# JARVIS-MoCap/JARVIS-HybridNet

Hardware: AMD Instinct MI355X
Metric: multi-view frames/s (12cam 1280x1024, 23kpt, 64^3 grid) (higher is better)
Workload: dtype f32; 1 GPU; BASELINE configs[2]: HybridNet 12-camera 1280x1024, 23 kpts, 64^3 grid, small/small; cameras=12, joints=23, grid=64, streams=3, parallelism=single GPU, 3 time batches in flight on 3 HIP streams, hipgraph=False

## Files before the change

include/jarvis_hip.h:

```cpp
#ifndef JARVIS_HIP_H
#define JARVIS_HIP_H
#include <stdint.h>

#ifdef __cplusplus
extern "C" {
#endif

#define JH_ABI_VERSION 4

const char* jh_last_error(void);
int jh_abi_version(void);

#define JH_PRECISION_DEFAULT (-1)
#define JH_PRECISION_F32 0
#define JH_PRECISION_BF16X3 1
#define JH_PRECISION_BF16X3_WIDE 2
int jh_set_precision(int mode);
int jh_get_precision(void);

typedef struct jh_params jh_params;
int jh_params_create(jh_params** out);
int jh_params_set(jh_params* p, const char* key, const float* host, int64_t numel);
void jh_params_destroy(jh_params* p);

typedef struct jh_efftrack jh_efftrack;
int jh_efftrack_create(const jh_params* p, const char* prefix, int model_size, int joints, int n,
                       int h, int w, int want_res1, jh_efftrack** out);
int jh_efftrack_forward(jh_efftrack* net, const float* x_dev, float* res1_dev, float* res2_dev,
                        void* stream);
int64_t jh_efftrack_launches(const jh_efftrack* net);
void jh_efftrack_destroy(jh_efftrack* net);

typedef struct jh_v2v jh_v2v;
int jh_v2v_create(const jh_params* p, const char* prefix, int joints, int t, int g, jh_v2v** out);
int jh_v2v_forward(jh_v2v* net, const float* x_dev, float* y_dev, void* stream);
void jh_v2v_destroy(jh_v2v* net);
int jh_v2v_fold(int joints, int t, int g, int* folded);

int64_t jh_reproject_workspace_bytes(int cams, int joints, int hs, int grid_size);
int jh_reproject_forward(const float* heatmaps_padded_dev, int cams, int joints, int hs,
                         const int32_t* center3d_dev, const int32_t* center_hm_dev,
                         const float* cam_dev, const float* intr_dev, const float* dist_dev,
                         int grid_size, float grid_spacing, float* vol_dev, int32_t* idx_dev,
                         void* workspace_dev, int64_t workspace_bytes, void* stream);

int64_t jh_softargmax_workspace_bytes(int t, int joints, int gh);
int jh_softargmax(const float* v2v_out_dev, int t, int joints, int gh, float grid_spacing,
                  float roi_cube_size, const int32_t* center3d_dev, float* heatmap_final_dev,
                  float* points_dev, float* conf_dev, void* workspace_dev, int64_t workspace_bytes,
                  void* stream);

int jh_reproject_point(const float* points_dev, int npoints, int cams, const float* cam_dev,
                       const float* intr_dev, const float* dist_dev, float* uv_dev, void* stream);
int64_t jh_reconstruct_workspace_bytes(int cams);
int jh_reconstruct_point(const float* points2d_dev, const float* maxvals_dev, int cams,
                         const float* cam_dev, const float* intr_dev, const float* dist_dev,
                         float* point3d_dev, void* workspace_dev, int64_t workspace_bytes,
                         void* stream);

typedef struct jh_predictor jh_predictor;
typedef struct {
  int32_t num_cameras, num_joints;
  int32_t center_size;
  int32_t bbox;
  float roi_cube_size;
  float grid_spacing;
  int32_t center_model, kp_model;
  int32_t img_h, img_w;
  int32_t time_batch;
  int32_t time_batch_3d;
  int32_t cam_lo, cam_n;
  float mean[3], std[3];
  int32_t precision;
} jh_predictor_config;

int jh_predictor_create(const jh_params* center_params, const jh_params* hybrid_params,
                        const jh_predictor_config* cfg, jh_predictor** out);
void jh_predictor_destroy(jh_predictor* pr);
int64_t jh_predictor_launches(const jh_predictor* pr);
int64_t jh_predictor_device_bytes(const jh_predictor* pr);
int jh_predictor_precision(const jh_predictor* pr);

int jh_predictor_set_calibration(jh_predictor* pr, const float* cam_dev, const float* intr_dev,
                                 const float* dist_dev, void* stream);
int jh_predictor_set_calibration_frames(jh_predictor* pr, const float* cam_dev ,
                                        const float* intr_dev , const float* dist_dev ,
                                        void* stream);

int jh_predictor_set_centers(jh_predictor* pr, const float* centers_dev , void* stream);

// ... 193 lines not shown
```

jarvis-hybridnet_amd/_native.py:

```python
import ctypes
import math
import os
from typing import NamedTuple

import torch

_HERE = os.path.dirname(os.path.abspath(__file__))
LIB_PATH = os.environ.get("JH_LIBRARY_PATH") or os.path.join(_HERE, "libjarvis_hip.so")
_lib = None

c_void_p, c_int, c_float, c_int64 = ctypes.c_void_p, ctypes.c_int, ctypes.c_float, ctypes.c_int64
c_char_p = ctypes.c_char_p


class PredictorConfig(ctypes.Structure):
    _fields_ = [("num_cameras", ctypes.c_int32), ("num_joints", ctypes.c_int32),
                ("center_size", ctypes.c_int32), ("bbox", ctypes.c_int32),
                ("roi_cube_size", c_float), ("grid_spacing", c_float),
                ("center_model", ctypes.c_int32), ("kp_model", ctypes.c_int32),
                ("img_h", ctypes.c_int32), ("img_w", ctypes.c_int32),
                ("time_batch", ctypes.c_int32), ("time_batch_3d", ctypes.c_int32),
                ("cam_lo", ctypes.c_int32),
                ("cam_n", ctypes.c_int32), ("mean", c_float * 3), ("std", c_float * 3),
                ("precision", ctypes.c_int32)]
# ... 13 lines not shown
    _fields_ = [("image_stride", ctypes.c_int64), ("offset", ctypes.c_int64), ("pitch", ctypes.c_int64),
                ("pattern", ctypes.c_int32), ("reserved", ctypes.c_int32)]


assert ctypes.sizeof(SensorSurfaceStruct) == 32

class OpOperand(ctypes.Structure):
    _fields_ = [("in_sums_host", c_void_p), ("in_act", ctypes.c_int32), ("latency_class", ctypes.c_int32),
                ("want_stats", ctypes.c_int32), ("se_c", ctypes.c_int32), ("se_s", ctypes.c_int32),
                ("se_inv_hw", c_float), ("se_wr_host", c_void_p), ("se_br_host", c_void_p),
                ("se_we_host", c_void_p), ("se_be_host", c_void_p), ("se_pool_host", c_void_p)]


assert ctypes.sizeof(OpOperand) == 72

class SubjectsParamsStruct(ctypes.Structure):
    _fields_ = [("max_subjects", ctypes.c_int32), ("max_peaks", ctypes.c_int32), ("nms_radius", ctypes.c_int32),
                ("min_views", ctypes.c_int32), ("min_peak", c_float), ("max_error_px", c_float)]


assert ctypes.sizeof(SubjectsParamsStruct) == 24

ABI_VERSION = 4
assert ctypes.sizeof(PredictorConfig) == 84

_WORKSPACES = {}


def workspace(nbytes, device):
    key = (str(device), torch.cuda.current_stream(device).cuda_stream)
    bufs = _WORKSPACES.setdefault(key, [])
    if not bufs or bufs[-1].numel() < nbytes:
        bufs.append(torch.empty((max(int(nbytes), 256),), dtype=torch.uint8, device=device))
    return bufs[-1]


_SIGS = {
    "jh_last_error": (c_char_p, []),
    "jh_abi_version": (c_int, []),
    "jh_set_precision": (c_int, [c_int]),
    "jh_get_precision": (c_int, []),
    "jh_params_create": (c_int, [ctypes.POINTER(c_void_p)]),
    "jh_params_set": (c_int, [c_void_p, c_char_p, c_void_p, c_int64]),
    "jh_params_destroy": (None, [c_void_p]),
    "jh_efftrack_create": (c_int, [c_void_p, c_char_p, c_int, c_int, c_int, c_int, c_int, c_int,
                                   ctypes.POINTER(c_void_p)]),
    "jh_efftrack_forward": (c_int, [c_void_p, c_void_p, c_void_p, c_void_p, c_void_p]),
    "jh_efftrack_launches": (c_int64, [c_void_p]),
    "jh_efftrack_destroy": (None, [c_void_p]),
    "jh_v2v_create": (c_int, [c_void_p, c_char_p, c_int, c_int, c_int, ctypes.POINTER(c_void_p)]),
    "jh_v2v_forward": (c_int, [c_void_p, c_void_p, c_void_p, c_void_p]),
    "jh_v2v_destroy": (None, [c_void_p]),
    "jh_v2v_fold": (c_int, [c_int, c_int, c_int, ctypes.POINTER(c_int)]),
    "jh_reproject_workspace_bytes": (c_int64, [c_int, c_int, c_int, c_int]),
    "jh_reproject_forward": (c_int, [c_void_p, c_int, c_int, c_int, c_void_p, c_void_p, c_void_p,
                                     c_void_p, c_void_p, c_int, c_float, c_void_p, c_void_p,
                                     c_void_p, c_int64, c_void_p]),
    "jh_softargmax_workspace_bytes": (c_int64, [c_int, c_int, c_int]),
    "jh_softargmax": (c_int, [c_void_p, c_int, c_int, c_int, c_float, c_float, c_void_p, c_void_p,
                              c_void_p, c_void_p, c_void_p, c_int64, c_void_p]),
    "jh_softargmax_spread_workspace_bytes": (c_int64, [c_int, c_int, c_int]),
    "jh_softargmax_spread": (c_int, [c_void_p, c_int, c_int, c_int, c_float, c_float, c_void_p, c_void_p,
                                     c_void_p, c_void_p, c_void_p, c_void_p, c_void_p, c_void_p, c_int64, c_void_p]),
    "jh_predictor_set_spread": (c_int, [c_void_p, c_int]),
    "jh_predictor_get_spread": (c_int, [c_void_p, c_void_p, c_void_p, c_void_p, c_void_p]),
    "jh_predictor_debug_v2v": (c_int, [c_void_p, c_void_p, c_void_p]),
    "jh_reproject_point": (c_int, [c_void_p, c_int, c_int, c_void_p, c_void_p, c_void_p, c_void_p,
                                   c_void_p]),
    "jh_reconstruct_workspace_bytes": (c_int64, [c_int]),
    "jh_reconstruct_point": (c_int, [c_void_p, c_void_p, c_int, c_void_p, c_void_p, c_void_p,
                                     c_void_p, c_void_p, c_int64, c_void_p]),
    "jh_predictor_create": (c_int, [c_void_p, c_void_p, ctypes.POINTER(PredictorConfig),
                                    ctypes.POINTER(c_void_p)]),
    "jh_predictor_destroy": (None, [c_void_p]),
    "jh_predictor_set_graph_replay": (c_int, [c_void_p, c_int]),
    "jh_predictor_graph_replay": (c_int, [c_void_p]),
    "jh_predictor_launches": (c_int64, [c_void_p]),
    "jh_predictor_device_bytes": (c_int64, [c_void_p]),
    "jh_predictor_precision": (c_int, [c_void_p]),
    "jh_predictor_set_calibration": (c_int, [c_void_p, c_void_p, c_void_p, c_void_p, c_void_p]),
    "jh_predictor_set_calibration_frames": (c_int, [c_void_p, c_void_p, c_void_p, c_void_p, c_void_p]),
    "jh_predictor_set_centers": (c_int, [c_void_p, c_void_p, c_void_p]),
    "jh_predictor_stage_center": (c_int, [c_void_p, c_void_p, c_void_p, c_void_p]),
    "jh_predictor_stage_keypoints": (c_int, [c_void_p, c_void_p, c_void_p, c_void_p, c_void_p]),
    "jh_predictor_stage_3d": (c_int, [c_void_p, c_void_p, c_int, c_void_p, c_void_p, c_void_p,
                                      c_void_p]),
    "jh_predictor_stage_keypoints_gathered": (c_int, [c_void_p, c_void_p, c_int, c_void_p, c_int, c_void_p,
                                                      c_void_p]),
    "jh_predictor_stage_3d_blocks": (c_int, [c_void_p, c_void_p, c_int, c_int, c_int, c_int, c_void_p,
                                             c_void_p, c_void_p, c_void_p]),
    "jh_profile_begin": (c_int, []),
    "jh_profile_end": (c_int, [ctypes.POINTER(c_int)]),
    "jh_profile_get": (c_int, [c_int, c_char_p, c_int, ctypes.POINTER(ctypes.c_double),
                               ctypes.POINTER(ctypes.c_double), ctypes.POINTER(ctypes.c_double)]),
    "jh_predictor_forward": (c_int, [c_void_p, c_void_p, c_void_p, c_void_p, c_void_p, c_void_p]),
    "jh_predictor_stage_center_u8": (c_int, [c_void_p, c_void_p, c_void_p, c_void_p]),
    "jh_predictor_stage_keypoints_u8": (c_int, [c_void_p, c_void_p, c_void_p, c_void_p, c_void_p]),
    "jh_predictor_forward_u8": (c_int, [c_void_p, c_void_p, c_void_p, c_void_p, c_void_p, c_void_p]),
    "jh_predictor_forward_yuv": (c_int, [c_void_p, c_void_p, c_int, c_void_p, c_void_p, c_void_p, c_void_p]),
    "jh_yuv_surface_check": (c_int, [ctypes.POINTER(YuvSurfaceStruct), c_int, c_int]),
    "jh_predictor_forward_surface": (c_int, [c_void_p, c_void_p, ctypes.POINTER(YuvSurfaceStruct), c_void_p, c_void_p,
                                             c_void_p, c_void_p, c_void_p]),
    "jh_predictor2d_forward_surface": (c_int, [c_void_p, c_void_p, ctypes.POINTER(YuvSurfaceStruct), c_void_p,
                                               c_void_p, c_void_p, c_void_p]),
    "jh_op_yuv_surface_to_bgr": (c_int, [c_void_p, ctypes.POINTER(YuvSurfaceStruct), c_int, c_int, c_int, c_void_p,
                                         c_void_p]),
# ... 402 lines not shown
```

jarvis-hybridnet_amd/csrc/api.hip:

```cpp
#include <cstring>
#include <memory>
#include "../../include/jarvis_hip.h"
#include <cstdlib>
#include "nets.h"
#include "bifpn_node.h"
#include "views2d.h"
#include "subjects.h"

namespace jh {
static thread_local std::string g_err;
void set_error(const std::string& msg) { g_err = msg; }
}

using namespace jh;

struct jh_params { ParamMap map; };
struct jh_efftrack { EffTrackPlan plan; };
struct jh_v2v { V2VPlan plan; };

namespace {

struct Scratch {
  std::vector<void*> ptrs;
  ~Scratch() { for (void* p : ptrs) (void)hipFree(p); }
// ... 126 lines not shown
  return 0;
}
int jh_get_precision(void) { return precision_mode(); }

int jh_params_create(jh_params** out) {
  *out = new jh_params();
  return 0;
}
int jh_params_set(jh_params* p, const char* key, const float* host, int64_t numel) {
  JH_REQUIRE(p && key && host && numel >= 0, "bad argument");
  p->map[key] = std::vector<float>(host, host + numel);
  return 0;
}
void jh_params_destroy(jh_params* p) { delete p; }

int jh_efftrack_create(const jh_params* p, const char* prefix, int model_size, int joints, int n,
                       int h, int w, int want_res1, jh_efftrack** out) {
  JH_REQUIRE(p && out, "bad argument");
  std::unique_ptr<jh_efftrack> net(new jh_efftrack());
  if (net->plan.build(p->map, prefix ? prefix : "", model_size, joints, n, h, w, want_res1 != 0)) return 1;
  *out = net.release();
  return 0;
}
int jh_efftrack_forward(jh_efftrack* net, const float* x_dev, float* res1_dev, float* res2_dev,
                        void* stream) {
  hipStream_t s = static_cast<hipStream_t>(stream);
  JH_REQUIRE(net && x_dev && res2_dev, "bad argument");
  JH_REQUIRE(!res1_dev || net->plan.res1.p, "res1 requested from a network created with want_res1 = 0");
  if (launch_to_channel_last(x_dev, net->plan.input, s)) return 1;
  if (net->plan.run(s)) return 1;
  if (res1_dev && launch_from_channel_last(net->plan.res1, res1_dev, s)) return 1;
  return launch_from_channel_last(net->plan.heat, res2_dev, s);
}
int64_t jh_efftrack_launches(const jh_efftrack* net) { return (int64_t)net->plan.launches(); }
void jh_efftrack_destroy(jh_efftrack* net) { delete net; }

int jh_v2v_create(const jh_params* p, const char* prefix, int joints, int t, int g, jh_v2v** out) {
  JH_REQUIRE(p && out, "bad argument");
  std::unique_ptr<jh_v2v> net(new jh_v2v());
  if (net->plan.build(p->map, prefix ? prefix : "", joints, t, g)) return 1;
  *out = net.release();
  return 0;
}
int jh_v2v_forward(jh_v2v* net, const float* x_dev, float* y_dev, void* stream) {
  hipStream_t s = static_cast<hipStream_t>(stream);
  if (launch_to_channel_last(x_dev, net->plan.input, s)) return 1;
  if (net->plan.run(s)) return 1;
  return launch_from_channel_last(net->plan.output, y_dev, s);
}
void jh_v2v_destroy(jh_v2v* net) { delete net; }
int jh_v2v_fold(int joints, int t, int g, int* folded) {
  JH_REQUIRE(joints >= 1 && t >= 1 && g >= 4 && g % 4 == 0 && folded, "jh_v2v_fold: bad argument");
  *folded = v2v_fold_applies(joints, g) ? 1 : 0;
  return 0;
}

int64_t jh_reproject_workspace_bytes(int cams, int joints, int hs, int grid_size) {
  Carver c(nullptr, 0);
  ReproWs w;
  return (int64_t)carve_reproject(c, cams, joints, hs, grid_size, &w);
}

int jh_reproject_forward(const float* heatmaps_padded_dev, int cams, int joints, int hs,
                         const int32_t* center3d_dev, const int32_t* center_hm_dev,
                         const float* cam_dev, const float* intr_dev, const float* dist_dev,
                         int grid_size, float grid_spacing, float* vol_dev, int32_t* idx_dev,
                         void* workspace_dev, int64_t workspace_bytes, void* stream) {
  hipStream_t s = static_cast<hipStream_t>(stream);
  JH_REQUIRE(workspace_dev && workspace_bytes >= 0, "workspace (see jh_reproject_workspace_bytes)");
  JH_REQUIRE(grid_size > 0 && grid_size % 2 == 0, "grid size must be even");
  Carver c(workspace_dev, (size_t)workspace_bytes);
  ReproWs w;
  carve_reproject(c, cams, joints, hs, grid_size, &w);
  JH_REQUIRE(c.fits(), "workspace smaller than jh_reproject_workspace_bytes()");
  if (launch_to_channel_last(heatmaps_padded_dev, w.heat, s)) return 1;
  if (launch_reproject(Calib{cam_dev, intr_dev, dist_dev, 0}, center3d_dev, center_hm_dev, w.heat.p, w.coarse,
                       w.vol.p, idx_dev, 1, cams, grid_size, grid_spacing, hs, w.heat.Cp,
                       1, 0, nullptr, s)) return 1;
  return launch_from_channel_last(w.vol, vol_dev, s);
}

int64_t jh_softargmax_workspace_bytes(int t, int joints, int gh) {
  Carver c(nullptr, 0);
  SoftWs w;
  return (int64_t)carve_softargmax(c, t, joints, gh, &w);
}

int jh_softargmax(const float* v2v_out_dev, int t, int joints, int gh, float grid_spacing,
                  float roi_cube_size, const int32_t* center3d_dev, float* heatmap_final_dev,
                  float* points_dev, float* conf_dev, void* workspace_dev, int64_t workspace_bytes,
                  void* stream) {
  hipStream_t s = static_cast<hipStream_t>(stream);
  JH_REQUIRE(workspace_dev && workspace_bytes >= 0, "workspace (see jh_softargmax_workspace_bytes)");
  Carver c(workspace_dev, (size_t)workspace_bytes);
  SoftWs w;
  carve_softargmax(c, t, joints, gh, &w);
  JH_REQUIRE(c.fits(), "workspace smaller than jh_softargmax_workspace_bytes()");
  if (launch_to_channel_last(v2v_out_dev, w.x, s)) return 1;
  return launch_softargmax(w.x.p, center3d_dev, w.partial, w.pmax, points_dev, conf_dev,
                           heatmap_final_dev, t, joints, w.x.Cp, gh, grid_spacing, roi_cube_size, s);
}

int64_t jh_softargmax_spread_workspace_bytes(int t, int joints, int gh) {
  Carver c(nullptr, 0);
  SoftWs w;
  SoftargmaxSpread sp;
// ... 1440 lines not shown
```

jarvis-hybridnet_amd/csrc/conv_host.hip:

```cpp
#include <vector>
#include <cstring>
#include <algorithm>
#include "conv_mfma.h"

namespace jh {

ConvDesc conv_desc(int nd, int k, int stride, int pad, int cin, int cout) {
  ConvDesc d{};
  d.nd = nd; d.k = k; d.stride = stride; d.ostride = 1; d.nphase = 1;
  d.cin = cin; d.cout = cout;
  d.phase[0].pad[0] = (nd == 3) ? pad : 0;
  d.phase[0].pad[1] = pad; d.phase[0].pad[2] = pad;
  d.phase[0].ooff[0] = d.phase[0].ooff[1] = d.phase[0].ooff[2] = 0;
  return d;
}

ConvDesc deconv2d_k4s2p1_desc(int cin, int cout) {
  ConvDesc d{};
  d.nd = 2; d.k = 2; d.stride = 1; d.ostride = 2; d.nphase = 4;
  d.cin = cin; d.cout = cout;
  for (int py = 0; py < 2; ++py)
    for (int px = 0; px < 2; ++px) {
      ConvPhase& p = d.phase[py * 2 + px];
      p.pad[0] = 0; p.pad[1] = py ? 0 : 1; p.pad[2] = px ? 0 : 1;
// ... 67 lines not shown
              const int nbk = co / 16, nn = co % 16;
              const int lane = kq * 16 + nn;
              if (tap_paired)
                packed[((((size_t)(tap / 2)) * nk8 + kc8) * nb + nbk) * 256 + lane * 4 + (tap & 1) * 2 + j] = v;
              else if (window) {
                const int sub = (1 - d.phase[ph].ooff[1]) * 2 + (1 - d.phase[ph].ooff[2]);
                const int col = sub * cout_p + co;
                packed[(((size_t)tap * npair + kc8 / 2) * nbw + col / 16) * 256 + (kq * 16 + col % 16) * 4 +
                       (kc8 & 1) * 2 + j] = v;
              }
              else if (paired)
                packed[ph * phase_stride + (((size_t)tap * (nk8 / 2) + kc8 / 2) * nb + nbk) * 256 + lane * 4 + (kc8 & 1) * 2 + j] = v;
              else
                packed[ph * phase_stride + (((size_t)tap * nk8 + kc8) * nb + nbk) * 128 + lane * 2 + j] = v;
            }
        }
  }
  out->cin_p = cin_p; out->cout_p16 = cout_p16; out->layout = layout;
  out->phase_stride = tap_paired ? packed.size() : (window ? packed.size() / d.nphase : phase_stride);
  return upload_conv_weights(packed.data(), packed.size() * sizeof(float), b, d.cout, out);
}

int upload_conv_weights(const void* packed, size_t bytes, const float* b, int cout, ConvWeights* out) {
  out->bias = nullptr;
  JH_CHECK_HIP(hipMalloc(reinterpret_cast<void**>(&out->w), bytes));
  JH_CHECK_HIP(hipMemcpy(out->w, packed, bytes, hipMemcpyHostToDevice));
  if (!b) return 0;
  std::vector<float> bp(out->cout_p16, 0.f);
  std::memcpy(bp.data(), b, cout * sizeof(float));
  JH_CHECK_HIP(hipMalloc(&out->bias, bp.size() * sizeof(float)));
  JH_CHECK_HIP(hipMemcpy(out->bias, bp.data(), bp.size() * sizeof(float), hipMemcpyHostToDevice));
  return 0;
}

void free_conv_weights(ConvWeights* w) {
  if (w->w) (void)hipFree(w->w);
  if (w->bias) (void)hipFree(w->bias);
  w->w = w->bias = nullptr;
}

static int pick_nr(int nb, int taps, bool heavy_staging, long units) {
  const double stage = (heavy_staging ? 1.5 : 0.5) / (double)taps;
  const long slots = 512;
  int best = 1;
  double best_cost = 1e30;
  for (int nr = 4; nr >= 1; --nr) {
    const long groups = (nb + nr - 1) / nr;
    const double cost = (double)std::max(units * groups, slots) * (stage + nr);
    if (cost < best_cost - 1e-9) { best_cost = cost; best = nr; }
  }
  return best;
}

int launch_conv(const ConvDesc& d, const ConvWeights& w, const Act& x, const Act& y,
                const float* gate, double* stats, hipStream_t s, const InNorm* in, const SeGate* se) {
  JH_REQUIRE(x.Cp == w.cin_p || (x.Cp == 4 && w.cin_p == 8), "conv input channel padding mismatch");
  JH_REQUIRE(y.Cp == cpad(d.cout), "conv output channel padding mismatch");
  JH_REQUIRE(x.N == y.N, "batch mismatch");
  ConvArgs a{};
  a.x = x.p; a.y = y.p; a.w = w.w; a.bias = w.bias; a.gate = gate; a.stats = stats;
  if (in && in->stats) {
    a.in_stats = in->stats; a.in_inv = in->inv; a.in_act = in->act;
    a.nrm_floats = 2 * w.cin_p;
  }
  if (gate) a.nrm_floats += w.cin_p;
  if (se && se->pool) {
    JH_REQUIRE(!gate, "either a gate tensor or a gate recipe");
    a.se = *se;
    a.nrm_floats += w.cin_p + round_up(se->C, 4) + round_up(se->S, 4);
  }
  a.N = x.N; a.Din = x.D; a.Hin = x.H; a.Win = x.W; a.cin_p = w.cin_p; a.in_px = x.Cp;
  a.Dy = y.D; a.Hy = y.H; a.Wy = y.W; a.cout_p = y.Cp; a.cout_p16 = w.cout_p16;
  a.ostride = d.ostride; a.nphase = d.nphase; a.phase_stride = w.phase_stride; a.layout = w.layout;
  for (int p = 0; p < d.nphase; ++p) a.phase[p] = d.phase[p];
  if (d.ostride > 1) { a.Dout = x.D; a.Hout = x.H; a.Wout = x.W; }
  else conv_out_shape(d, x.D, x.H, x.W, &a.Dout, &a.Hout, &a.Wout);
  int Do, Ho, Wo;
  conv_out_shape(d, x.D, x.H, x.W, &Do, &Ho, &Wo);
  JH_REQUIRE(Do == y.D && Ho == y.H && Wo == y.W, "conv output extent mismatch");
  const int taps = d.k * d.k * (d.nd == 3 ? d.k : 1);
  long units;
  if (d.nd == 2) units = (long)((a.Hout + 7) / 8) * ((a.Wout <= 8 ? a.Wout + 7 : a.Wout + 15) / (a.Wout <= 8 ? 8 : 16));
  else units = (long)((a.Dout + 1) / 2) * ((a.Hout + 3) / 4) * ((a.Wout + 15) / 16);
  units *= (long)a.nphase * a.N;
  const int nr = pick_nr(w.cout_p16 / 16, taps, (in && in->stats && in->act == ACT_SILU) || gate || (se && se->pool),
                         units);
  const size_t budget = kConvLdsBudget;
  switch (w.layout) {
    case WeightLayout::Window: return launch_deconv4_window(a, s);
    case WeightLayout::ChannelPaired: return launch_deconv4_fused(a, s);
    case WeightLayout::TapPaired: case WeightLayout::Plain: break;
  }
  if (conv_pw_direct_eligible(d, a)) return launch_conv_pw_direct(a, s);
  if (d.nd == 2) {
    const int small = (a.Wout <= 8) ? 1 : 0;
    const int big = (a.Wout >= 64 && a.Hout >= 64 && w.cin_p <= 32 && d.ostride == 1 && d.stride == 1 &&
               (d.k == 1 || d.k == 3)) ? 1 : 0;
    if (big) return conv_launch_2d_big(a, d.k, d.stride, nr, budget, s);
    if (d.k == 1 && d.stride == 1 && d.ostride == 1 && d.nphase == 1 && (a.Wout % 16 != 0 || a.Hout % 8 != 0) &&
        a.Hout * a.Wout >= 96 && a.Hin == a.Hout && a.Win == a.Wout && a.Hy == a.Hout && a.Wy == a.Wout) {
      ConvArgs f = a;
      f.Win = f.Wout = f.Wy = a.Hout * a.Wout;
      f.Hin = f.Hout = f.Hy = 1;
      return conv_launch_2d_k1_flat(f, nr, budget, s);
    }
    if (d.k == 1 && d.stride == 1) return conv_launch_2d_k1(a, nr, small, budget, s);
    if (d.k == 2 && d.stride == 1) return conv_launch_2d_k2(a, nr, small, budget, s);
    if (d.k == 3 && d.stride == 1 && d.ostride == 1 && a.Wout > 16 && a.Wout <= 20 && a.Hout <= 22 &&
        !d.latency_class)
      return conv_launch_2d_k3_w20(a, nr, std::max(budget, (size_t)64 * 1024), s);
    if (!d.latency_class && d.ostride == 1) {
      if (d.k == 5 && d.stride <= 2 && a.Wout > 32 && a.Wout <= 40)
        return conv_launch_2d_k5_w40(a, d.stride, nr, std::max(budget, (size_t)64 * 1024), s);
      if (d.k == 3 && d.stride == 2 && a.Wout > 16 && a.Wout <= 20 && a.Hout <= 22)
        return conv_launch_2d_k3s2_w20(a, nr, std::max(budget, (size_t)96 * 1024), s);
    }
    if (d.k == 3 && d.stride <= 2) return conv_launch_2d_k3(a, d.stride, nr, small, budget, s);
    if (d.k == 5 && d.stride <= 2) return conv_launch_2d_k5(a, d.stride, nr, small, budget, s);
  } else {
    const int nr_form = pick_nr(w.cout_p16 / 16, taps,
                                (in && in->stats && in->act == ACT_SILU) || gate || (se && se->pool), 1L << 40);
    const long tiles_big = (long)((a.Dout + 1) / 2) * ((a.Hout + 3) / 4) * ((a.Wout + 15) / 16) *
                           a.nphase * ((w.cout_p16 / 16 + nr_form - 1) / nr_form);
    int small = tiles_big < 16 ? 1 : 0;
    if (!small && d.k == 3 && d.stride == 1 && tiles_big >= 256) small = 2;
    if (d.k == 1 && d.stride == 1) return conv_launch_3d_k1(a, nr, small, budget, s);
    if (d.k == 2 && d.stride == 2) return conv_launch_3d_k2s2(a, nr, small, budget, s);
    if (d.k == 3 && d.stride <= 2) return conv_launch_3d_k3(a, d.stride, nr, small, budget, s);
  }
  JH_REQUIRE(false, "no convolution kernel for this (nd, k, stride)");
}

}
```

jarvis-hybridnet_amd/csrc/conv_mfma.h:

```cpp
#pragma once
#include <cstdlib>
#include <type_traits>
#include "jh_common.h"

namespace jh {

typedef float f32x4 __attribute__((ext_vector_type(4)));

template <int ND, int K, int STRIDE, int TZ, int TY, int TX>
struct ConvGeom {
  static constexpr int KD = (ND == 3) ? K : 1;
  static constexpr int KH = K, KW = K;
  static constexpr int NT = KD * KH * KW;
  static constexpr int PZ = (TZ - 1) * STRIDE + KD;
  static constexpr int PY = (TY - 1) * STRIDE + KH;
  static constexpr int PX = (TX - 1) * STRIDE + KW;
  static constexpr int NPIX = PZ * PY * PX;
  static constexpr int TM = TZ * TY * TX;
  static constexpr int MR = TM / 64;
  static constexpr int SPAD = (STRIDE == 1) ? 4 : 2;
  static_assert(TM % 64 == 0 || (TZ == 1 && TM / 64 >= 1), "tile must cover at least 64 pixels");
  static size_t lds_bytes(int kc) { return (size_t)NPIX * (kc + SPAD) * sizeof(float); }
};

// ... 530 lines not shown
        for (int nr = 0; nr < NR; ++nr) bn[k8][nr] = wload(koff[k8], nr);
      int tap = 0;
      for (int dz = 0; dz < G::KD; ++dz)
        for (int dy = 0; dy < G::KH; ++dy) {
          const int row_off = (dz * G::PY + dy) * G::PX * S2;
#pragma unroll
          for (int dx = 0; dx < G::KW; ++dx, ++tap) {
            float2 bc[KC8][NR], ac[KC8][MR];
#pragma unroll
            for (int k8 = 0; k8 < KC8; ++k8)
#pragma unroll
              for (int mr = 0; mr < MR; ++mr) ac[k8][mr] = lds2[abase[mr] + row_off + dx * S2 + k8 * 4];
            const int wn = min(tap + 1, G::NT - 1) * tap_stride;
#pragma unroll
            for (int k8 = 0; k8 < KC8; ++k8)
#pragma unroll
              for (int nr = 0; nr < NR; ++nr) {
                bc[k8][nr] = bn[k8][nr];
                bn[k8][nr] = wload(wn + koff[k8], nr);
              }
#pragma unroll
            for (int k8 = 0; k8 < KC8; ++k8) {
#pragma unroll
              for (int mr = 0; mr < MR; ++mr)
#pragma unroll
                for (int nr = 0; nr < NR; ++nr)
                  acc[mr][nr] = __builtin_amdgcn_mfma_f32_16x16x4f32(ac[k8][mr].x, bc[k8][nr].x, acc[mr][nr], 0, 0, 0);
#pragma unroll
              for (int mr = 0; mr < MR; ++mr)
#pragma unroll
                for (int nr = 0; nr < NR; ++nr)
                  acc[mr][nr] = __builtin_amdgcn_mfma_f32_16x16x4f32(ac[k8][mr].y, bc[k8][nr].y, acc[mr][nr], 0, 0, 0);
            }
          }
        }
      }
    }
  }

  __syncthreads();
  EpilogueArgs e;
  e.y = a.y + (size_t)n * a.Dy * a.Hy * a.Wy * a.cout_p;
  e.bias = a.bias;
  e.stats = a.stats ? a.stats + (size_t)n * a.cout_p * kStatW : nullptr;
  e.Dout = a.Dout; e.Hout = a.Hout; e.Wout = a.Wout; e.Hy = a.Hy; e.Wy = a.Wy;
  e.cout_p = a.cout_p; e.cout_p16 = a.cout_p16; e.os = a.ostride; e.osz = a.ostride;
  e.offz = a.phase[ph].ooff[0]; e.offy = a.phase[ph].ooff[1]; e.offx = a.phase[ph].ooff[2];
  if (oz0 + TZ <= a.Dout && oy0 + TY <= a.Hout && ox0 + TX <= a.Wout)
    conv_epilogue<MR, NR, TY, TX, 4, true>(acc, e, lds, nb0, oz0, oy0, ox0, tid);
  else
    conv_epilogue<MR, NR, TY, TX>(acc, e, lds, nb0, oz0, oy0, ox0, tid);
}

constexpr size_t kConvLdsBudget = 40 * 1024;

inline int pick_kc8(int cin_p, size_t (*lds_bytes)(int), size_t budget) {
  int best = 1;
  double best_cost = 1e30;
  for (int k = 1; k <= 4; ++k) {
    if (lds_bytes(k * 8) > budget && k > 1) continue;
    const int chunks = (cin_p + k * 8 - 1) / (k * 8);
    const double cost = (double)chunks * k * 8 / cin_p + 0.02 * chunks;
    if (cost < best_cost - 1e-9) { best_cost = cost; best = k; }
  }
  return best;
}

template <int ND, int K, int STRIDE, int TZ, int TY, int TX, int NRV, int KC8V>
int launch_conv_inst(const ConvArgs& b, dim3 grid, hipStream_t s) {
  using G = ConvGeom<ND, K, STRIDE, TZ, TY, TX>;
  size_t lds = G::lds_bytes(KC8V * 8);
  const size_t red = (size_t)4 * 4 * 16 * 2 * sizeof(double);
  if (lds < red) lds = red;
  lds += (size_t)b.nrm_floats * sizeof(float);
  JH_REQUIRE(lds <= 160 * 1024, "conv patch does not fit LDS");
  auto kern = conv_mfma_kernel<ND, K, STRIDE, TZ, TY, TX, NRV, KC8V>;
  static bool big_lds_enabled = false;
  if (lds > 64 * 1024 && !big_lds_enabled) {
    JH_CHECK_HIP(hipFuncSetAttribute(reinterpret_cast<const void*>(kern),
                                     hipFuncAttributeMaxDynamicSharedMemorySize, 160 * 1024));
    big_lds_enabled = true;
  }
  ConvArgs c = b;
  c.fgx = make_fastdiv(grid.x); c.fgy = make_fastdiv(grid.y);
  c.ftx = make_fastdiv((b.Wout + TX - 1) / TX); c.fty = make_fastdiv((b.Hout + TY - 1) / TY);
  JH_REQUIRE(b.nphase == 1 || b.nphase == 4 || b.nphase == 8, "phase count");
  hipLaunchKernelGGL(kern, grid, dim3(256), lds, s, c);
  JH_CHECK_HIP(hipGetLastError());
  return 0;
}

template <int ND, int K, int STRIDE, int TZ, int TY, int TX>
int launch_conv_geom(const ConvArgs& a, int nr, size_t lds_budget, hipStream_t s) {
  using G = ConvGeom<ND, K, STRIDE, TZ, TY, TX>;
  ConvArgs b = a;
  const int kc8 = pick_kc8(b.cin_p, &G::lds_bytes, lds_budget);
  b.kc = kc8 * 8;
  const int tiles = ((b.Dout + TZ - 1) / TZ) * ((b.Hout + TY - 1) / TY) * ((b.Wout + TX - 1) / TX);
  const int nb = b.cout_p16 / 16;
  while (nr > 1 && (long)tiles * ((nb + nr - 1) / nr) * b.N * b.nphase <= 128) --nr;
  dim3 grid(tiles, (nb + nr - 1) / nr, b.N * b.nphase);
#define JH_CONV_CASE(NRV, KV) \
  if (nr == NRV && kc8 == KV) return launch_conv_inst<ND, K, STRIDE, TZ, TY, TX, NRV, KV>(b, grid, s);
#define JH_CONV_ROW(NRV) JH_CONV_CASE(NRV, 1) JH_CONV_CASE(NRV, 2) JH_CONV_CASE(NRV, 3) JH_CONV_CASE(NRV, 4)
  JH_CONV_ROW(1) JH_CONV_ROW(2) JH_CONV_ROW(3) JH_CONV_ROW(4)
#undef JH_CONV_ROW
// ... 27 lines not shown
```

jarvis-hybridnet_amd/csrc/jh_common.h:

```cpp
#pragma once
#include <hip/hip_runtime.h>
#include <cstdlib>
#include <cstdint>
#include <cstdio>
#include <cstring>
#include <string>
#include <vector>

namespace jh {

constexpr int kWave = 64;

#define JH_ENV_KNOB(name) ([]() -> int { static const int v = [] { const char* e = getenv(name); return e ? atoi(e) : -1; }(); return v; }())

inline int round_up(int v, int m) { return (v + m - 1) / m * m; }
inline int cpad(int c) { return round_up(c, 8); }

void set_error(const std::string& msg);
#define JH_CHECK_HIP(expr)                                                     \
  do {                                                                         \
    hipError_t _e = (expr);                                                    \
    if (_e != hipSuccess) {                                                    \
      jh::set_error(std::string(#expr) + ": " + hipGetErrorString(_e));        \
      return 1;                                                                \
// ... 87 lines not shown
  f.d = d;
  unsigned l = 0;
  while ((1ull << l) < d) ++l;
  f.shift = l;
  f.mul = (unsigned)((((1ull << l) - d) << 32) / d + 1);
  return f;
}

struct SeGate {
  const double* pool = nullptr;
  const float *wr = nullptr, *br = nullptr, *we = nullptr, *be = nullptr;
  int C = 0, S = 0;
  float inv_hw = 0.f;
};

struct ConvArgs {
  const float* x;
  float* y;
  const float* w;
  const float* bias;
  const float* gate;
  SeGate se;
  const double* in_stats;
  float in_inv;
  int in_act;
  int nrm_floats;
  double* stats;
  int N, Din, Hin, Win, cin_p;
  int Dout, Hout, Wout;
  int Dy, Hy, Wy, cout_p;
  int cout_p16;
  int kc;
  int in_px;
  int ostride, nphase;
  WeightLayout layout = WeightLayout::Plain;
  FastDiv fgx, fgy, ftx, fty;
  size_t phase_stride;
  ConvPhase phase[8];
};

int pack_conv_weights(const ConvDesc& d, const float* w_host, const float* b_host,
                      bool transposed, WeightLayout layout, ConvWeights* out);
int upload_conv_weights(const void* packed, size_t bytes, const float* b, int cout, ConvWeights* out);
void free_conv_weights(ConvWeights* w);

struct InNorm {
  const double* stats = nullptr;
  float inv = 0.f;
  int act = 0;
};
int launch_conv(const ConvDesc& d, const ConvWeights& w, const Act& x, const Act& y,
                const float* gate, double* stats, hipStream_t s, const InNorm* in = nullptr,
                const SeGate* se = nullptr);
void conv_out_shape(const ConvDesc& d, int D, int H, int W, int* Do, int* Ho, int* Wo);

ConvDesc conv_desc(int nd, int k, int stride, int pad, int cin, int cout);
ConvDesc deconv2d_k4s2p1_desc(int cin, int cout);
ConvDesc deconv3d_k2s2_desc(int cin, int cout);
long deconv4_window_launches();

int launch_norm_apply(const Act& x, const double* stats, double eps, int act,
                      const float* r1, const float* r2, float* y, double* pool,
                      hipStream_t s, const double* r1_stats = nullptr, int min_block_kb = 0);
int launch_se_gate(const double* pool, int N, int C, int Cp, int S, float inv_hw,
                   const float* wr, const float* br, const float* we, const float* be,
                   float* gate, hipStream_t s);
bool depthwise_can_pool(int H, int W);
int launch_depthwise(const Act& x, const float* w, int k, float* y, double* stats,
                     hipStream_t s, double* pool = nullptr);
enum FuseMode { FUSE_SAME = 0, FUSE_UP2 = 1, FUSE_UP4 = 2, FUSE_POOL2 = 3 };
struct FuseArgs {
  const float* in[3];
  int mode[3];
  float w[3];
  int n_in;
  int act;
};
int launch_fuse(const FuseArgs& f, const Act& out, hipStream_t s);
int launch_maxpool2(const Act& x, float* y, hipStream_t s);

struct BlockId { unsigned x, y, z; };

constexpr int kLimbs = 3;
constexpr int kStatW = 2 * kLimbs;
#if defined(__HIPCC__)
__device__ __forceinline__ void exact_add(double* dst, double p) {
  const double h = rint(p * 0x1p-16) * 0x1p16;
  const double r = p - h;
  const double m = rint(r * 0x1p20) * 0x1p-20;
  const double l = rint((r - m) * 0x1p56) * 0x1p-56;
  if (h != 0.0) unsafeAtomicAdd(dst + 0, h);
  if (m != 0.0) unsafeAtomicAdd(dst + 1, m);
  if (l != 0.0) unsafeAtomicAdd(dst + 2, l);
}
__device__ __forceinline__ double exact_read(const double* src) { return (src[0] + src[1]) + src[2]; }
__device__ __forceinline__ void stat_add(double* st, float s1, float s2) {
  exact_add(st, (double)s1);
  exact_add(st + kLimbs, (double)s2);
}
__device__ __forceinline__ void exact_add_rounded(double* dst, double p) {
  const double a = fabs(p);
  double q;
  int slot;
  if (a < 0x1p5) { q = rint(p * 0x1p35) * 0x1p-35; slot = 2; }
  else if (a < 0x1p15) { q = rint(p * 0x1p25) * 0x1p-25; slot = 1; }
  else { q = rint(p * 0x1p15) * 0x1p-15; slot = 0; }
// ... 115 lines not shown
```

Measured before the change: 2195 multi-view frames/s.

## Add tile-walking 2D conv kernel that keeps weights in registers across row tiles

Adds a new MFMA 3x3 2D conv kernel where each block walks several consecutive tiles along a row. It loads the weights into registers once and prefetches the next input patch while computing the current one, optionally double-buffered in LDS. It is used for specific small-channel shapes (stride 1 with cin 16, and stride 2 with cin 8 and 48 outputs) when the batch is large enough. Walk length comes from a grid-size heuristic and can be set with an environment knob. The gain is less weight reloading and more overlap of loads with compute, at the cost of fewer blocks in flight, higher register pressure and added code paths.

```diff
diff --git a/include/jarvis_hip.h b/include/jarvis_hip.h
--- a/include/jarvis_hip.h
+++ b/include/jarvis_hip.h
@@ -36,6 +36,8 @@
 int jh_v2v_forward(jh_v2v* net, const float* x_dev, float* y_dev, void* stream);
 void jh_v2v_destroy(jh_v2v* net);
 int jh_v2v_fold(int joints, int t, int g, int* folded);
+
+int jh_conv_walk(int k, int stride, int cin, int cout, int h, int w, int n, int gated, int* walk);
 
 int64_t jh_reproject_workspace_bytes(int cams, int joints, int hs, int grid_size);
 int jh_reproject_forward(const float* heatmaps_padded_dev, int cams, int joints, int hs,
diff --git a/jarvis-hybridnet_amd/_native.py b/jarvis-hybridnet_amd/_native.py
--- a/jarvis-hybridnet_amd/_native.py
+++ b/jarvis-hybridnet_amd/_native.py
@@ -89,6 +89,7 @@
     "jh_v2v_forward": (c_int, [c_void_p, c_void_p, c_void_p, c_void_p]),
     "jh_v2v_destroy": (None, [c_void_p]),
     "jh_v2v_fold": (c_int, [c_int, c_int, c_int, ctypes.POINTER(c_int)]),
+    "jh_conv_walk": (c_int, [c_int] * 8 + [ctypes.POINTER(c_int)]),
     "jh_reproject_workspace_bytes": (c_int64, [c_int, c_int, c_int, c_int]),
     "jh_reproject_forward": (c_int, [c_void_p, c_int, c_int, c_int, c_void_p, c_void_p, c_void_p,
                                      c_void_p, c_void_p, c_int, c_float, c_void_p, c_void_p,
diff --git a/jarvis-hybridnet_amd/csrc/api.hip b/jarvis-hybridnet_amd/csrc/api.hip
--- a/jarvis-hybridnet_amd/csrc/api.hip
+++ b/jarvis-hybridnet_amd/csrc/api.hip
@@ -202,6 +202,13 @@
 int jh_v2v_fold(int joints, int t, int g, int* folded) {
   JH_REQUIRE(joints >= 1 && t >= 1 && g >= 4 && g % 4 == 0 && folded, "jh_v2v_fold: bad argument");
   *folded = v2v_fold_applies(joints, g) ? 1 : 0;
+  return 0;
+}
+
+int jh_conv_walk(int k, int stride, int cin, int cout, int h, int w, int n, int gated, int* walk) {
+  JH_REQUIRE(k >= 1 && (stride == 1 || stride == 2) && cin >= 1 && cout >= 1 && h >= 1 && w >= 1 && n >= 1 && walk,
+             "jh_conv_walk: bad argument");
+  *walk = conv_walk_query(k, stride, cin, cout, h, w, n, gated != 0);
   return 0;
 }
 
diff --git a/jarvis-hybridnet_amd/csrc/conv_host.hip b/jarvis-hybridnet_amd/csrc/conv_host.hip
--- a/jarvis-hybridnet_amd/csrc/conv_host.hip
+++ b/jarvis-hybridnet_amd/csrc/conv_host.hip
@@ -143,6 +143,51 @@
   return best;
 }
 
+static bool conv_big_tiles(const ConvDesc& d, const ConvArgs& a) {
+  return a.Wout >= 64 && a.Hout >= 64 && a.cin_p <= 32 && d.ostride == 1 && d.stride == 1 &&
+         (d.k == 1 || d.k == 3);
+}
+
+bool conv_walk_eligible(const ConvDesc& d, const ConvArgs& a) {
+  if (d.nd != 2 || d.k != 3 || d.ostride != 1 || d.nphase != 1 || a.layout != WeightLayout::Plain) return false;
+  if (a.gate || a.se.pool || a.in_px != a.cin_p) return false;
+  const int nb = a.cout_p16 / 16;
+  if (d.stride == 1) return a.cin_p == 16 && nb == 1 && conv_big_tiles(d, a);
+  if (d.stride == 2)
+    return a.cin_p == 8 && nb == 3 && a.Wout > 8 &&
+           !(!d.latency_class && a.Wout > 16 && a.Wout <= 20 && a.Hout <= 22);
+  return false;
+}
+
+int conv_walk_length(const ConvDesc& d, const ConvArgs& a) {
+  const char* env = getenv("JH_CONV_WALK");
+  const int knob = env ? atoi(env) : 1;
+  if (knob <= 0 || !conv_walk_eligible(d, a)) return 0;
+  const int tiles_x = (a.Wout + 15) / 16, tiles_y = (a.Hout + (d.stride == 1 ? 15 : 7)) / (d.stride == 1 ? 16 : 8);
+  if (knob >= 2) {
+    int w = std::min(knob, 8);
+    while (w > 1 && tiles_x % w != 0) w >>= 1;
+    return w;
+  }
+  if (a.N <= 32) return 0;
+  const long want = 4 * 256;
+  for (const int w : {tiles_x, 4, 2})
+    if (w >= 1 && tiles_x % w == 0 && (long)a.N * tiles_y * (tiles_x / w) >= want) return w;
+  return 1;
+}
+
+int conv_walk_query(int k, int stride, int cin, int cout, int H, int W, int N, bool gated) {
+  const ConvDesc d = conv_desc(2, k, stride, k / 2, cin, cout);
+  static const float some_gate = 0.f;
+  ConvArgs a{};
+  a.gate = gated ? &some_gate : nullptr;
+  a.N = N; a.Din = 1; a.Hin = H; a.Win = W; a.cin_p = a.in_px = cpad(cin);
+  a.cout_p = cpad(cout); a.cout_p16 = round_up(cout, 16);
+  a.ostride = 1; a.nphase = 1; a.layout = WeightLayout::Plain;
+  conv_out_shape(d, 1, H, W, &a.Dout, &a.Hout, &a.Wout);
+  return conv_walk_length(d, a);
+}
+
 int launch_conv(const ConvDesc& d, const ConvWeights& w, const Act& x, const Act& y,
                 const float* gate, double* stats, hipStream_t s, const InNorm* in, const SeGate* se) {
   JH_REQUIRE(x.Cp == w.cin_p || (x.Cp == 4 && w.cin_p == 8), "conv input channel padding mismatch");
@@ -183,11 +228,10 @@
     case WeightLayout::TapPaired: case WeightLayout::Plain: break;
   }
   if (conv_pw_direct_eligible(d, a)) return launch_conv_pw_direct(a, s);
+  if (const int walk = conv_walk_length(d, a)) return conv_launch_2d_walk(a, d.stride, walk, s);
   if (d.nd == 2) {
     const int small = (a.Wout <= 8) ? 1 : 0;
-    const int big = (a.Wout >= 64 && a.Hout >= 64 && w.cin_p <= 32 && d.ostride == 1 && d.stride == 1 &&
-               (d.k == 1 || d.k == 3)) ? 1 : 0;
-    if (big) return conv_launch_2d_big(a, d.k, d.stride, nr, budget, s);
+    if (conv_big_tiles(d, a)) return conv_launch_2d_big(a, d.k, d.stride, nr, budget, s);
     if (d.k == 1 && d.stride == 1 && d.ostride == 1 && d.nphase == 1 && (a.Wout % 16 != 0 || a.Hout % 8 != 0) &&
         a.Hout * a.Wout >= 96 && a.Hin == a.Hout && a.Win == a.Wout && a.Hy == a.Hout && a.Wy == a.Wout) {
       ConvArgs f = a;
diff --git a/jarvis-hybridnet_amd/csrc/conv_mfma.h b/jarvis-hybridnet_amd/csrc/conv_mfma.h
--- a/jarvis-hybridnet_amd/csrc/conv_mfma.h
+++ b/jarvis-hybridnet_amd/csrc/conv_mfma.h
@@ -606,6 +606,210 @@
     conv_epilogue<MR, NR, TY, TX>(acc, e, lds, nb0, oz0, oy0, ox0, tid);
 }
 
+template <int ND, int K, int STRIDE, int TZ, int TY, int TX, int NR, int KC8, bool DB>
+__global__ __launch_bounds__(256, DB ? 3 : 4) void conv_mfma_walk_kernel(const ConvArgs a, const int walk) {
+  static_assert(ND == 2 && TZ == 1, "the tile walk is a 2D form");
+  using G = ConvGeom<ND, K, STRIDE, TZ, TY, TX>;
+  constexpr int MR = G::MR;
+  constexpr int KC = KC8 * 8, S = KC + G::SPAD, S2 = S / 2, Q4 = KC / 4;
+  constexpr int BUF2 = G::NPIX * S2;
+  constexpr int RED = 4 * NR * 16 * 2 * 2;
+  constexpr int ITER = (G::NPIX * Q4 + 255) / 256;
+  static_assert(256 % Q4 == 0, "all patch items of a thread share one channel quad");
+  extern __shared__ __attribute__((aligned(16))) float lds_all[];
+  float* nrm = lds_all;
+  float* red = lds_all + a.nrm_floats;
+  float2* patch2 = reinterpret_cast<float2*>(red + RED);
+
+  const int tid = threadIdx.x;
+  const int lane = tid & 63;
+  const int wave = __builtin_amdgcn_readfirstlane(tid >> 6);
+  const int mrow = lane & 15;
+  const int kq = lane >> 4;
+
+  const BlockId bid = xcd_block(a.fgx, a.fgy);
+  const int runs_x = (int)a.ftx.d;
+  const int tile_y = (int)fd_div(bid.x, a.ftx);
+  const int tile_x0 = ((int)bid.x - tile_y * runs_x) * walk;
+  const int nb0 = bid.y * NR;
+  const int n = bid.z;
+  const int oy0 = tile_y * TY;
+  const int iy0 = oy0 * STRIDE - a.phase[0].pad[1];
+
+  int abase[MR];
+#pragma unroll
+  for (int mr = 0; mr < MR; ++mr) {
+    const int p = (wave * MR + mr) * 16 + mrow;
+    const int tx = p % TX, ty = p / TX;
+    abase[mr] = ((ty * STRIDE) * G::PX + tx * STRIDE) * S2 + kq;
+  }
+
+  if (a.in_stats) {
+    for (int c = tid; c < a.cin_p; c += 256) {
+      const double* st = a.in_stats + ((size_t)n * a.cin_p + c) * kStatW;
+      const double mu = exact_read(st) * (double)a.in_inv;
+      double var = exact_read(st + kLimbs) * (double)a.in_inv - mu * mu;
+      if (var < 0.0) var = 0.0;
+      nrm[c] = (float)mu;
+      nrm[a.cin_p + c] = (float)(1.0 / sqrt(var + 1e-5));
+    }
+  }
+
+  const int nkc8_total = a.cin_p >> 3;
+  const int nb16_total = a.cout_p16 >> 4;
+  const int tap_stride = nkc8_total * nb16_total * 64;
+  const __amdgpu_buffer_rsrc_t wrs = __builtin_amdgcn_make_buffer_rsrc(
+      const_cast<float*>(a.w), 0, (int)(a.phase_stride * 4), 0x00020000);
+  typedef unsigned int wu2 __attribute__((ext_vector_type(2)));
+  float2 breg[G::NT][KC8][NR];
+#pragma unroll
+  for (int nr = 0; nr < NR; ++nr) {
+    const int wvo = (min(nb0 + nr, nb16_total - 1) * 64 + lane) * 8;
+#pragma unroll
+    for (int tp = 0; tp < G::NT; ++tp)
+#pragma unroll
+      for (int k8 = 0; k8 < KC8; ++k8) {
+        const wu2 v = __builtin_amdgcn_raw_buffer_load_b64(
+            wrs, wvo, (tp * tap_stride + min(k8, nkc8_total - 1) * nb16_total * 64) * 8, 0);
+        breg[tp][k8][nr] = make_float2(__uint_as_float(v.x), __uint_as_float(v.y));
+      }
+  }
+
+  const float* __restrict__ xin = a.x + (size_t)n * a.Hin * a.Win * a.in_px;
+  const __amdgpu_buffer_rsrc_t xrs = __builtin_amdgcn_make_buffer_rsrc(
+      const_cast<float*>(xin), 0, (int)((size_t)a.Hin * a.Win * a.in_px * 4), 0x00020000);
+  typedef float cf4 __attribute__((ext_vector_type(4)));
+  float4 pf[ITER];
+  unsigned okm = 0;
+  auto issue_tile = [&](int tile_x, int t) __attribute__((always_inline)) {
+    const int ix0 = tile_x * TX * STRIDE - a.phase[0].pad[2];
+    okm = 0;
+#pragma unroll
+    for (int it = 0; it < ITER; ++it) {
+      const int pix = t / Q4 + it * (256 / Q4);
+      const int ix = ix0 + pix % G::PX, iy = iy0 + pix / G::PX;
+      const bool ok = t + it * 256 < G::NPIX * Q4 && iy >= 0 && iy < a.Hin && ix >= 0 && ix < a.Win;
+      const int off = ok ? ((iy * a.Win + ix) * a.in_px + (t % Q4) * 4) * 4 : (int)0x80000000;
+      okm |= (ok ? 1u : 0u) << it;
+      const cf4 v = __builtin_bit_cast(cf4, __builtin_amdgcn_raw_buffer_load_b128(xrs, off, 0, 0));
+      pf[it] = make_float4(v[0], v[1], v[2], v[3]);
+    }
+  };
+  const int mode = !a.in_stats ? 0 : (a.in_act == ACT_RELU ? 2 : (a.in_act == ACT_SILU ? 3 : 1));
+  auto commit_tile = [&](float2* dst2, auto mode_c) __attribute__((always_inline)) {
+    constexpr int MODE = decltype(mode_c)::value;
+    float4 mu = make_float4(0.f, 0.f, 0.f, 0.f), rs = make_float4(1.f, 1.f, 1.f, 1.f);
+    if (MODE != 0) {
+      mu = *reinterpret_cast<const float4*>(nrm + (tid % Q4) * 4);
+      rs = *reinterpret_cast<const float4*>(nrm + a.cin_p + (tid % Q4) * 4);
+    }
+#pragma unroll
+    for (int it = 0; it < ITER; ++it) {
+      const int idx = tid + it * 256;
+      if (idx < G::NPIX * Q4) {
+        const int c4 = tid % Q4, pix = tid / Q4 + it * (256 / Q4);
+        float4 v = pf[it];
+        if (MODE != 0) {
+          const float m = ((okm >> it) & 1u) ? 1.f : 0.f;
+          v.x = (v.x - mu.x) * rs.x; v.y = (v.y - mu.y) * rs.y;
+          v.z = (v.z - mu.z) * rs.z; v.w = (v.w - mu.w) * rs.w;
+          if (MODE == 2) {
+            v.x = fmaxf(v.x, 0.f); v.y = fmaxf(v.y, 0.f); v.z = fmaxf(v.z, 0.f); v.w = fmaxf(v.w, 0.f);
+          } else if (MODE == 3) {
+            v.x = silu_fast(v.x); v.y = silu_fast(v.y);
+            v.z = silu_fast(v.z); v.w = silu_fast(v.w);
+          }
+          v.x *= m; v.y *= m; v.z *= m; v.w *= m;
+        }
+        float2* dst = dst2 + pix * S2 + c4 * 2;
+        dst[0] = make_float2(v.x, v.y);
+        dst[1] = make_float2(v.z, v.w);
+      }
+    }
+  };
+
+  EpilogueArgs e;
+  e.y = a.y + (size_t)n * a.Dy * a.Hy * a.Wy * a.cout_p;
+  e.bias = a.bias;
+  e.stats = a.stats ? a.stats + (size_t)n * a.cout_p * kStatW : nullptr;
+  e.Dout = a.Dout; e.Hout = a.Hout; e.Wout = a.Wout; e.Hy = a.Hy; e.Wy = a.Wy;
+  e.cout_p = a.cout_p; e.cout_p16 = a.cout_p16; e.os = a.ostride; e.osz = a.ostride;
+  e.offz = a.phase[0].ooff[0]; e.offy = a.phase[0].ooff[1]; e.offx = a.phase[0].ooff[2];
+
+  issue_tile(tile_x0, tid);
+  __syncthreads();
+  for (int i = 0; i < walk; ++i) {
+    float2* cur2 = patch2 + (DB ? (i & 1) * BUF2 : 0);
+    if (!DB && i > 0) __syncthreads();
+    if (mode == 0) commit_tile(cur2, std::integral_constant<int, 0>{});
+    else if (mode == 3) commit_tile(cur2, std::integral_constant<int, 3>{});
+    else if (mode == 2) commit_tile(cur2, std::integral_constant<int, 2>{});
+    else commit_tile(cur2, std::integral_constant<int, 1>{});
+    __syncthreads();
+    int t = tid;
+    asm volatile("" : "+v"(t));
+    if (i + 1 < walk) issue_tile(tile_x0 + i + 1, t);
+
+    f32x4 acc[MR][NR];
+#pragma unroll
+    for (int mr = 0; mr < MR; ++mr)
+#pragma unroll
+      for (int nr = 0; nr < NR; ++nr) acc[mr][nr] = (f32x4){0.f, 0.f, 0.f, 0.f};
+#pragma unroll
+    for (int tp = 0; tp < G::NT; ++tp) {
+      const int toff = ((tp / G::KW) * G::PX + tp % G::KW) * S2;
+      float2 ac[KC8][MR];
+#pragma unroll
+      for (int k8 = 0; k8 < KC8; ++k8)
+#pragma unroll
+        for (int mr = 0; mr < MR; ++mr) ac[k8][mr] = cur2[abase[mr] + toff + k8 * 4];
+#pragma unroll
+      for (int k8 = 0; k8 < KC8; ++k8) {
+#pragma unroll
+        for (int mr = 0; mr < MR; ++mr)
+#pragma unroll
+          for (int nr = 0; nr < NR; ++nr)
+            acc[mr][nr] = __builtin_amdgcn_mfma_f32_16x16x4f32(ac[k8][mr].x, breg[tp][k8][nr].x, acc[mr][nr], 0, 0, 0);
+#pragma unroll
+        for (int mr = 0; mr < MR; ++mr)
+#pragma unroll
+          for (int nr = 0; nr < NR; ++nr)
+            acc[mr][nr] = __builtin_amdgcn_mfma_f32_16x16x4f32(ac[k8][mr].y, breg[tp][k8][nr].y, acc[mr][nr], 0, 0, 0);
+      }
+    }
+
+    const int ox0 = (tile_x0 + i) * TX;
+    if (oy0 + TY <= a.Hout && ox0 + TX <= a.Wout)
+      conv_epilogue<MR, NR, TY, TX, 4, true>(acc, e, red, nb0, 0, oy0, ox0, t);
+    else
+      conv_epilogue<MR, NR, TY, TX>(acc, e, red, nb0, 0, oy0, ox0, t);
+  }
+}
+
+bool conv_walk_eligible(const ConvDesc& d, const ConvArgs& a);
+int conv_walk_length(const ConvDesc& d, const ConvArgs& a);
+int conv_launch_2d_walk(const ConvArgs& a, int stride, int walk, hipStream_t s);
+
+template <int ND, int K, int STRIDE, int TZ, int TY, int TX, int NRV, int KC8V, bool DB>
+int launch_conv_walk_inst(const ConvArgs& b, int walk, hipStream_t s) {
+  using G = ConvGeom<ND, K, STRIDE, TZ, TY, TX>;
+  const int tiles_x = (b.Wout + TX - 1) / TX, tiles_y = (b.Hout + TY - 1) / TY, nb = b.cout_p16 / 16;
+  JH_REQUIRE(walk >= 1 && tiles_x % walk == 0, "conv walk: the walk divides the tiles of a row");
+  JH_REQUIRE(b.cin_p == KC8V * 8 && b.in_px == b.cin_p && !b.gate && !b.se.pool && b.nphase == 1,
+             "conv walk: shape (conv_walk_eligible)");
+  const size_t lds = (size_t)b.nrm_floats * sizeof(float) + (size_t)4 * NRV * 16 * 2 * sizeof(double) +
+                     (DB ? 2 : 1) * G::lds_bytes(KC8V * 8);
+  JH_REQUIRE(lds <= 64 * 1024, "conv walk: LDS");
+  const dim3 grid(tiles_y * (tiles_x / walk), (nb + NRV - 1) / NRV, b.N);
+  ConvArgs c = b;
+  c.kc = KC8V * 8;
+  c.fgx = make_fastdiv(grid.x); c.fgy = make_fastdiv(grid.y);
+  c.ftx = make_fastdiv(tiles_x / walk); c.fty = make_fastdiv(tiles_y);
+  hipLaunchKernelGGL((conv_mfma_walk_kernel<ND, K, STRIDE, TZ, TY, TX, NRV, KC8V, DB>), grid, dim3(256), lds, s, c, walk);
+  JH_CHECK_HIP(hipGetLastError());
+  return 0;
+}
+
 constexpr size_t kConvLdsBudget = 40 * 1024;
 
 inline int pick_kc8(int cin_p, size_t (*lds_bytes)(int), size_t budget) {
diff --git a/jarvis-hybridnet_amd/csrc/conv_tu_2d_walk.hip b/jarvis-hybridnet_amd/csrc/conv_tu_2d_walk.hip
--- /dev/null
+++ b/jarvis-hybridnet_amd/csrc/conv_tu_2d_walk.hip
@@ -0,0 +1,8 @@
+#include "conv_mfma.h"
+namespace jh {
+int conv_launch_2d_walk(const ConvArgs& a, int stride, int walk, hipStream_t s) {
+  if (stride == 1) return launch_conv_walk_inst<2, 3, 1, 1, 16, 16, 1, 2, false>(a, walk, s);
+  if (stride == 2) return launch_conv_walk_inst<2, 3, 2, 1, 8, 16, 3, 1, true>(a, walk, s);
+  JH_REQUIRE(false, "no tile-walking kernel for this conv");
+}
+}
diff --git a/jarvis-hybridnet_amd/csrc/jh_common.h b/jarvis-hybridnet_amd/csrc/jh_common.h
--- a/jarvis-hybridnet_amd/csrc/jh_common.h
+++ b/jarvis-hybridnet_amd/csrc/jh_common.h
@@ -163,6 +163,7 @@
 int launch_conv(const ConvDesc& d, const ConvWeights& w, const Act& x, const Act& y,
                 const float* gate, double* stats, hipStream_t s, const InNorm* in = nullptr,
                 const SeGate* se = nullptr);
+int conv_walk_query(int k, int stride, int cin, int cout, int H, int W, int N, bool gated);
 void conv_out_shape(const ConvDesc& d, int D, int H, int W, int* Do, int* Ho, int* Wo);
 
 ConvDesc conv_desc(int nd, int k, int stride, int pad, int cin, int cout);
```

Result: no change. 2192 multi-view frames/s (-0.1%).
